# MrTornado24/FENeRF

Measured on AMD Instinct MI355X. Metric: rays/s/GPU forward render (128x128, 24+24 samples, H=256 FiLM-SIREN + 32x96^3 grid), higher is better.
Workload: dtype f16x3 (error-compensated fp16 MFMA, fp32 accumulate; fp32-class accuracy); 1 GPU; configs[1]: CelebA_double_semantic_texture_embedding_256_dim_96 generator, 128x128, 24+24 hierarchical samples, batch 1/GPU, forward-only render, procedural weights; img_size=128, num_steps=24, batch_per_gpu=1

## Files before the change

fenerf_amd/_lib.py:

```python
import ctypes as C
import os

import numpy as np

_HERE = os.path.dirname(os.path.abspath(__file__))
LIB_PATH = os.environ.get("FENERF_LIB", os.path.join(_HERE, "libfenerf_hip.so"))

ABI_VERSION = 2
MAX_GEO, MAX_COLOR, MAX_LABEL = 8, 4, 3

OK, E_INVALID, E_HIP, E_NOMEM, E_UNSUPPORTED, E_CLAMP_MODE = 0, -1, -2, -3, -4, -5
CLAMP = {"relu": 1, "softplus": 2}
FILL = {None: 0, "weight": 1, "seg_padding_background": 2, "eval_seg_padding_background": 3, "eval_white_back": 4}
FILL_COLORS = {"white": 1.0, "black": 0.0, "grey": 0.5, "light_grey": 0.81}

_fp = C.POINTER(C.c_float)
_vp = C.c_void_p


class FenerfModelDesc(C.Structure):
    _fields_ = [
        ("abi_version", C.c_int32), ("hidden_dim", C.c_int32), ("n_geo", C.c_int32), ("n_color", C.c_int32),
        ("n_label_layers", C.c_int32), ("output_dim", C.c_int32), ("grid_ch", C.c_int32),
        ("grid_d", C.c_int32), ("grid_h", C.c_int32), ("grid_w", C.c_int32), ("box_scale", C.c_float),
# ... 115 lines not shown
    "fenerf_siren_forward_save_pointwise": (_i, [_vp, _i, _i64] + [_vp] * 10),
    "fenerf_siren_backward_pointwise": (_i, [_vp, _i, _i64] + [_vp] * 9 + [_i, _vp]),
    "fenerf_siren_param_grads_pointwise": (_i, [_vp, _i, _i64] + [_vp] * 10 + [C.POINTER(FenerfSirenGrads)] + [_vp] * 2 + [_i, _vp]),
    "fenerf_siren_param_grads_fmt": (_i, [_vp, _i, _i64] + [_vp] * 9 + [_i, _vp, _vp, C.POINTER(FenerfSirenGrads), C.POINTER(FenerfSirenGrads)] + [_vp] * 3),
    "fenerf_siren_backward_stream_bytes_fmt": (_i, [_vp, _i64, _i, C.POINTER(C.c_double)]),
    "fenerf_model_set_forward_mode": (_i, [_vp, _i]),
    "fenerf_render_save_bytes": (_sz, [_vp, _i, _i, _i, _i, _i]),
    "fenerf_render_forward_save": (_i, [_vp, _i, _i, _i, _i] + [_vp] * 10 + [C.POINTER(FenerfCompositeOpts), _vp, _vp, _vp, _sz, _i, _vp]),
    "fenerf_render_backward_workspace_bytes": (_sz, [_vp, _i, _i, _i, _i, _i64, _i64]),
    "fenerf_render_backward": (_i, [_vp, _i, _i, _i, _i, _vp, _sz, _i, _vp, _vp, C.POINTER(FenerfCompositeOpts), _vp, C.POINTER(FenerfSirenGrads), _vp,
                                    C.POINTER(FenerfSirenGrads), _i64, _i64, _vp, _sz, _vp]),
    "fenerf_render_backward_split_workspace_bytes": (_sz, [_vp, _i, _i, _i, _i64, _i]),
    "fenerf_render_backward_stage": (_i, [_vp, _i, _i, _i, _i, _i, _i, _vp, _sz, _i, _vp, _vp, C.POINTER(FenerfCompositeOpts), _vp, C.POINTER(FenerfSirenGrads), _vp,
                                          C.POINTER(FenerfSirenGrads), _i64, _vp, _sz, _vp]),
    "fenerf_ray_grads": (_i, [_i, _i, _i, _i] + [_vp] * 7),
    "fenerf_render_backward_rays_workspace_bytes": (_sz, [_vp, _i, _i, _i, _i, _i, _i64, _i64]),
    "fenerf_render_backward_rays": (_i, [_vp, _i, _i, _i, _i, _vp, _sz, _i, _vp, _vp, C.POINTER(FenerfCompositeOpts), _vp, C.POINTER(FenerfSirenGrads), _vp,
                                         C.POINTER(FenerfSirenGrads), _i64, _i64, _vp, _sz, _vp, _vp, _i, _vp, _vp, _vp]),
    "fenerf_composite_backward_outputs": (_i, [_i64, _i, _i, _i, _vp, _vp, _vp, _vp, _vp, C.POINTER(FenerfCompositeOpts)] + [_vp] * 7),
    "fenerf_render_backward_outputs": (_i, [_vp, _i, _i, _i, _i, _vp, _sz, _i, _vp, _vp, C.POINTER(FenerfCompositeOpts), _vp, _vp, C.POINTER(FenerfSirenGrads),
                                            _vp, C.POINTER(FenerfSirenGrads), _i64, _i64, _vp, _sz, _vp, _vp, _i, _vp, _vp, _vp]),
    "fenerf_sparse_select_workspace_bytes": (C.c_size_t, [_i, _i64]),
    "fenerf_sparse_select": (_i, [_i, _i, _i, _i, _i64, _vp, _vp, _vp, _vp, _vp, _vp, _vp, _vp, _vp, _vp, _vp, _vp, C.c_size_t, _vp]),
    "fenerf_mesh_workspace_bytes": (_sz, [_i, _i, _i]),
    "fenerf_mesh_count": (_i, [_vp, _i, _i, _i, C.c_float, _vp, _vp, _vp]),
    "fenerf_mesh_emit": (_i, [_vp, _i, _i, _i, C.c_float, C.POINTER(C.c_float), C.POINTER(C.c_float), _vp, _i64, _i64, _vp, _vp, _vp]),
    "fenerf_volume_components_workspace_bytes": (_sz, [_i, _i, _i]),
    "fenerf_volume_components": (_i, [_vp, _i, _i, _i, C.c_float, _vp, _vp, _vp, _vp]),
    "fenerf_volume_keep_components": (_i, [_vp, _vp, _vp, _i, _i, _i, _i, _i64, _vp, _vp]),
    "fenerf_mesh_cluster_workspace_bytes": (_sz, [_i64, _i64, _i, _i, _i, _i]),
    "fenerf_mesh_cluster_count": (_i, [_vp, _i64, _vp, _i64, C.POINTER(C.c_float), C.POINTER(C.c_float), _i, _i, _i, _i, _vp, _vp, _vp]),
    "fenerf_mesh_cluster_emit": (_i, [_vp, _i64, _i64, C.POINTER(C.c_float), C.POINTER(C.c_float), _i, _i, _i, _i, _vp, _i64, _i64, _vp, _vp, _vp]),
    "fenerf_volume_sample": (_i, [_vp, _i, _i, _i, _i, _i, C.POINTER(C.c_float), C.POINTER(C.c_float), C.c_float, _i64, _vp, _vp, _vp]),
    "fenerf_volume_sample_rays": (_i, [_vp, _i, _i, _i, _i, _i, C.POINTER(C.c_float), C.POINTER(C.c_float), C.c_float, _i, _i, _i, _vp, _vp, _vp, _vp, _vp]),
    "fenerf_volume_render_workspace_bytes": (_sz, [_i, _i, _i, _i, _i]),
    "fenerf_volume_render": (_i, [_vp, _i, _i, _i, _i, _i, C.POINTER(C.c_float), C.POINTER(C.c_float), C.c_float, _i, _i, _i, _i] + [_vp] * 6 +
                             [C.POINTER(FenerfCompositeOpts)] + [_vp] * 4 + [_vp, _sz, _vp]),
    "fenerf_surface_points": (_i, [_i, _i, _vp, _vp, _vp, _vp, C.c_float, _vp, _vp]),
    "fenerf_volume_sample_grad": (_i, [_vp, _i, _i, _i, _i, _i, C.POINTER(C.c_float), C.POINTER(C.c_float), _i64, _vp, _vp, _vp]),
    "fenerf_shade_normals": (_i, [_i, _i, _i64, _vp, _vp, _vp, C.POINTER(C.c_float), C.c_float, C.c_float, C.c_float, _vp, _vp, _vp]),
    "fenerf_composite_backward": (_i, [_i64, _i, _i, _i, _vp, _vp, _vp, _vp, _vp, C.POINTER(FenerfCompositeOpts), _vp, _vp, _vp, _vp]),
    "fenerf_render_workspace_bytes": (_sz, [_vp, _i, _i, _i, _i]),
    "fenerf_render_forward": (_i, [_vp, _i, _i, _i, _i, _i] + [_vp] * 10 + [C.POINTER(FenerfCompositeOpts)] + [_vp] * 4 + [_vp, _sz, _vp]),
}
EXPORTS = tuple(_SIGS)
N_PHASES = 19
# ... 163 lines not shown
```

fenerf_amd/csrc/fenerf_api.cpp:

```cpp
#include <hip/hip_runtime.h>

#include <atomic>
#include <cmath>
#include <cstddef>
#include <cstdio>
#include <cstdlib>
#include <cstring>
#include <map>
#include <mutex>
#include <new>
#include <string>
#include <vector>

#include "fenerf_internal.h"

namespace fenerf {
static thread_local std::string g_err;
void set_error(const std::string& msg) { g_err = msg; }

int fail(int code, const std::string& msg) {
  set_error(msg);
  return code;
}
int hip_fail(hipError_t e, const char* what) {
// ... 1099 lines not shown
  p.BR = BR; p.M = M; p.C = C; p.N = N;
  p.rows_a = rows_a; p.rows_b = rows_b; p.z_a = z_a; p.z_b = z_b; p.noise = noise; p.o = *opts;
  p.g_rgb = g_rgb; p.d_rows_a = d_rows_a; p.d_rows_b = d_rows_b;
  const CompositeOutGrads g{g_depth, g_weights, g_wsum};
  { PhaseScope ph(PH_COMPOSITE_BWD, stream); return launch_composite_backward_outputs(p, g, merge != 0, stream); }
}

extern "C" size_t fenerf_sparse_select_workspace_bytes(int B, int64_t P) {
  if (B < 1 || P < 1) return 0;
  return sparse_select_workspace_bytes(B, P);
}

extern "C" int fenerf_sparse_select(int B, int R, int N, int C, int64_t cap, const float* d_coarse, const float* d_fine, const float* z_coarse,
                                    const float* z_fine, const float* origins, const float* dirs, const int64_t* images, float* pts, float* rd,
                                    float* d_sel, int32_t* counts, void* workspace, size_t workspace_bytes, void* stream) {
  if (B < 1 || B > 65535 || R < 1 || N < 1 || C < 1 || cap < 1) return fail(FENERF_E_INVALID, "need 1 <= B <= 65535, R, N, C, cap >= 1");
  if ((int64_t)R * N > (int64_t)1 << 36) return fail(FENERF_E_INVALID, "too many samples per image");
  if (!d_coarse || !z_coarse || !origins || !dirs || !pts || !d_sel || !counts || !workspace || (!d_fine) != (!z_fine))
    return fail(FENERF_E_INVALID, "NULL pointer (d_fine and z_fine may be NULL together: one pass)");
  if (workspace_bytes < sparse_select_workspace_bytes(B, (int64_t)R * N)) return fail(FENERF_E_INVALID, "workspace too small (fenerf_sparse_select_workspace_bytes)");
  { PhaseScope ph(PH_OTHER, stream); return launch_sparse_select(B, R, N, C, cap, d_coarse, d_fine, z_coarse, z_fine, origins, dirs, (const long long*)images, pts, rd, d_sel, counts, workspace, stream); }
}

namespace {
int check_lattice(const char* who, int n0, int n1, int n2) {
  if (n0 < 2 || n1 < 2 || n2 < 2) return fail(FENERF_E_INVALID, std::string(who) + ": every lattice axis needs at least 2 points");
  if ((int64_t)n0 * n1 * n2 > INT32_MAX) return fail(FENERF_E_INVALID, std::string(who) + ": more than 2^31 - 1 lattice points");
  return FENERF_OK;
}
}

extern "C" size_t fenerf_mesh_workspace_bytes(int n0, int n1, int n2) {
  if (check_lattice("fenerf_mesh_workspace_bytes", n0, n1, n2) != FENERF_OK) return 0;
  return mesh_workspace_bytes(n0, n1, n2);
}

extern "C" int fenerf_mesh_count(const float* vol, int n0, int n1, int n2, float iso, void* workspace, int64_t* counts_dev, void* stream) {
  if (int rc = check_lattice("fenerf_mesh_count", n0, n1, n2)) return rc;
  if (!vol || !workspace || !counts_dev) return fail(FENERF_E_INVALID, "fenerf_mesh_count: vol / workspace / counts_dev is NULL");
  { PhaseScope ph(PH_OTHER, stream); return launch_mesh_count(vol, n0, n1, n2, iso, workspace, (long long*)counts_dev, stream); }
}

extern "C" int fenerf_mesh_emit(const float* vol, int n0, int n1, int n2, float iso, const float origin[3], const float spacing[3], const void* workspace,
                                int64_t n_vertices, int64_t n_faces, float* vertices, int32_t* faces, void* stream) {
  if (int rc = check_lattice("fenerf_mesh_emit", n0, n1, n2)) return rc;
  if (!vol || !workspace || !origin || !spacing) return fail(FENERF_E_INVALID, "fenerf_mesh_emit: vol / workspace / origin / spacing is NULL");
// ... 173 lines not shown
  float* wts = (float*)(base + ws.wts);
  float* zf = (float*)(base + ws.zf);
  cp.BR = BR; cp.M = N; cp.C = C; cp.N = N;
  cp.rows_a = coarse; cp.z_a = z_coarse; cp.noise = noise_coarse;
  cp.o.clamp_mode = opts->clamp_mode; cp.o.noise_std = opts->noise_std;
  cp.out_weights = wts;
  cp.out_ch = C - 1; cp.sigma_only = 1;
  rc = run_composite(cp, false, stream);
  if (rc) return rc;
  { PhaseScope ph(PH_RESAMPLE, stream); rc = launch_resample(BR, N, z_coarse, wts, u, zf, stream); }
  if (rc) return rc;
  rc = run_volume_rays(vp, BR, N, origins, dirs, zf, fine, stream);
  if (rc) return rc;
  memset(&cp, 0, sizeof(cp));
  cp.BR = BR; cp.M = 2 * N; cp.C = C; cp.N = N;
  cp.rows_a = fine; cp.rows_b = coarse; cp.z_a = zf; cp.z_b = z_coarse; cp.noise = noise_final; cp.o = *opts;
  cp.out_rgb = out_rgb; cp.out_depth = out_depth; cp.out_weights = out_weights; cp.out_wsum = out_wsum;
  cp.out_ch = out_channels(C, opts);
  return run_composite(cp, true, stream);
}

namespace {
struct RenderWs {
  size_t film, coarse, fine, wts, zf, counts, idx, xbuf, total;
};
RenderWs render_ws(const FenerfModel* m, int B, int R, int N, int hier) {
  RenderWs w;
  const size_t pts = (size_t)B * R * N;
  size_t off = 0;
  w.film = off; off += fenerf_film_workspace_bytes(m, B);
  w.coarse = off; off += align_up(pts * m->C * sizeof(float), 256);
  w.fine = off; off += hier ? align_up(pts * m->C * sizeof(float), 256) : 0;
  w.wts = off; off += hier ? align_up(pts * sizeof(float), 256) : 0;
  w.zf = off; off += hier ? align_up(pts * sizeof(float), 256) : 0;
  const bool split = hier && m->precision == FENERF_PREC_F16X3;
  w.counts = off; off += split ? align_up((size_t)B * sizeof(unsigned), 256) : 0;
  w.idx = off; off += split ? align_up(pts * sizeof(unsigned), 256) : 0;
  w.xbuf = off; off += split ? align_up(pts * (size_t)m->H * sizeof(float), 256) : 0;
  w.total = off;
  return w;
}
}

extern "C" size_t fenerf_render_workspace_bytes(const FenerfModel* m, int B, int R, int N, int hierarchical) {
  if (!m || B <= 0 || R <= 0 || N <= 0) return 0;
  return render_ws(m, B, R, N, hierarchical).total;
}

extern "C" int fenerf_render_forward(const FenerfModel* m, int B, int R, int N, int hierarchical, int lock_view,
                                     const float* origins, const float* dirs, const float* z_coarse, const float* u,
                                     const float* noise_coarse, const float* noise_final, const float* freq_geo,
                                     const float* phase_geo, const float* freq_app, const float* phase_app,
                                     const FenerfCompositeOpts* opts, float* out_rgb, float* out_depth,
                                     float* out_weights, float* out_wsum, void* workspace, size_t workspace_bytes,
                                     void* stream) {
  if (!m) return fail(FENERF_E_INVALID, "model is NULL");
  int rc = check_opts(opts);
  if (rc) return rc;
  if (B <= 0 || R <= 0 || N <= 0) return fail(FENERF_E_INVALID, "B, R, N must be > 0");
  const int M = hierarchical ? 2 * N : N;
// ... 38 lines not shown
    c1.rows_a = coarse; c1.z_a = z_coarse; c1.noise = noise_coarse;
    c1.o.clamp_mode = opts->clamp_mode; c1.o.noise_std = opts->noise_std;
    c1.sigma_only = 1; c1.out_ch = m->C - 1;
    c1.u = u; c1.z_fine = zf;
    memset(&c2, 0, sizeof(c2));
    c2.BR = BR; c2.M = 2 * N; c2.C = m->C; c2.N = N;
    c2.rows_a = fine; c2.rows_b = coarse; c2.z_a = zf; c2.z_b = z_coarse; c2.noise = noise_final; c2.o = *opts;
    c2.out_rgb = out_rgb; c2.out_depth = out_depth; c2.out_weights = out_weights; c2.out_wsum = out_wsum;
    c2.out_ch = out_channels(m->C, opts);
    sp.out = coarse;
    PhaseScope ph(PH_RENDER_FUSED, stream);
    return launch_render16w_fused(m, sp, plan, zf, fine, c1, c2, stream);
  }
  const bool split_ok = m->precision == FENERF_PREC_F16X3 && m->forward_mode == FENERF_FORWARD_F16X3 && opts->clamp_mode == FENERF_CLAMP_RELU &&
                        !opts->last_back && (opts->noise_std == 0.f || !noise_final) && m->d_colour_nonfinite;
  if (g_render_split == FENERF_SPLIT_FORCE && !split_ok)
    return fail(FENERF_E_UNSUPPORTED, "fenerf_set_render_split(FORCE): the density + colour route needs an f16x3 model at its default forward mode, "
                                      "the relu clamp, last_back off and no noise on the final composite");
  const bool split = split_ok && (g_render_split == FENERF_SPLIT_FORCE || (g_render_split == FENERF_SPLIT_AUTO && kSplitAutoEnabled));
  SplitArgs sa;
  memset(&sa, 0, sizeof(sa));
  if (split) {
    sa.counts = (unsigned*)(base + ws.counts); sa.idx = (unsigned*)(base + ws.idx); sa.xbuf = (float*)(base + ws.xbuf);
    sa.cap = (long long)R * N; sa.keep_all = m->d_colour_nonfinite;
    HIP_TRY(hipMemsetAsync(sa.counts, 0, (size_t)B * sizeof(unsigned), (hipStream_t)stream));
    rc = [&] { PhaseScope ph(PH_SIREN, stream); PhaseScope pd(PH_SIREN_DENSITY, stream); return launch_siren16w_density(m, sp, sa, stream); }();
  } else {
    rc = run_siren(m, sp, stream);
  }
  if (rc) return rc;
  sp.raw_fg = nullptr;
  memset(&cp, 0, sizeof(cp));
  cp.BR = BR; cp.M = N; cp.C = m->C; cp.N = N;
  cp.rows_a = coarse; cp.z_a = z_coarse; cp.noise = noise_coarse;
  cp.o.clamp_mode = opts->clamp_mode; cp.o.noise_std = opts->noise_std;
  cp.sigma_only = 1; cp.out_ch = m->C - 1;
  cp.u = u; cp.z_fine = zf;
  rc = run_composite(cp, false, stream);
  if (rc) return rc;
  if (split) {
    rc = [&] { PhaseScope ph(PH_SIREN_COLOUR, stream); return launch_siren16w_colour(m, sp, sa, stream); }();
    if (rc) return rc;
  }
  sp.z = zf; sp.out = fine;
  rc = run_siren(m, sp, stream);
  if (rc) return rc;
  memset(&cp, 0, sizeof(cp));
  cp.BR = BR; cp.M = 2 * N; cp.C = m->C; cp.N = N;
// ... 557 lines not shown
```

fenerf_amd/csrc/fenerf_internal.h:

```cpp
#pragma once
#include <hip/hip_runtime_api.h>

#include <cstddef>
#include <cstdint>
#include <map>
#include <mutex>
#include <string>
#include <vector>

#include "../../include/fenerf.h"
#include "fenerf_layout.h"

namespace fenerf {

void set_error(const std::string& msg);
int fail(int code, const std::string& msg);
int hip_fail(hipError_t e, const char* what);
int check_launch(const char* what);
int ensure_dynamic_lds(const void* kfn, size_t bytes);
enum Phase { PH_FILM_PREP = 0, PH_SIREN, PH_SIREN_SAVE, PH_CHAIN, PH_WGRAD_FILM, PH_WGRAD_SQ, PH_WGRAD_SQ_REDUCE, PH_WGRAD_THIN,
             PH_WGRAD_THIN_REDUCE, PH_COMPOSITE, PH_RESAMPLE, PH_COMPOSITE_BWD, PH_REPACK, PH_GRID, PH_RAY_SETUP, PH_OTHER, PH_RENDER_FUSED,
             PH_SIREN_DENSITY, PH_SIREN_COLOUR, PH_COUNT };
static_assert(PH_COUNT == FENERF_N_PHASES_ALL && PH_RENDER_FUSED + 1 == FENERF_N_PHASES, "include/fenerf.h FENERF_N_PHASES / FENERF_N_PHASES_ALL");
struct PhaseScope {
// ... 125 lines not shown
int launch_siren_backward(const FenerfModel* m, const SirenBwdParams& p, void* stream);
int launch_siren_backward16w(const FenerfModel* m, const SirenBwdParams& p, void* stream);
bool use_bf16_dump(const FenerfModel* m, long long total_points);
int bwd16w_film_unit(long long total_points, long long pts_per_image);
size_t wgrad_workspace_bytes(const FenerfModel* m, int B, long long P);
int launch_param_grads(const FenerfModel* m, int B, long long P, const float* points, const float* dirs, const float* fp, const float* pp,
                       const float* out, const float* d_out, const float* tape, const float* tape_e, const float* d_t,
                       const FenerfSirenGrads& g, bool film_only, void* workspace, void* stream, const float* film_tiles = nullptr,
                       int tape_format = 0, const FenerfSirenGrads* weights = nullptr,
                       int film_per_point = 0);
int launch_grid_backward(const FenerfModel* m, long long P, const float* points, const float* d_e, float* d_grid_cl, void* stream);
size_t grid_det_workspace_bytes(const FenerfModel* m);
int launch_grid_backward_det(const FenerfModel* m, long long rows, long long dense_rows, const float* points, const float* d_e, float* out,
                             bool to_ncdhw, void* workspace, void* stream);
int launch_siren_input_grads(const FenerfModel* m, int B, long long P, const float* points, const float* fp, const float* d_t, const float* w_geo0,
                             const float* w_color0, int w_color0_ld, float* d_points, float* d_dirs, void* stream);
int launch_ray_grads(int B, int R, int N, long long Pp, int passes, const float* d_pts2, const float* d_rd2, const float* z_coarse,
                     const float* z_fine, float* d_origins, float* d_dirs, void* stream);
int launch_siren16w(const FenerfModel* m, const SirenParams& p, void* stream);
struct SplitArgs {
  unsigned* counts;
  unsigned* idx;
  float* xbuf;
  long long cap;
  const unsigned* keep_all;
};
int launch_siren16w_density(const FenerfModel* m, const SirenParams& p, const SplitArgs& s, void* stream);
int launch_siren16w_colour(const FenerfModel* m, const SirenParams& p, const SplitArgs& s, void* stream);
int launch_nonfinite_scan(FenerfModel* m, bool grid_too, void* stream);
struct FusedRenderPlan { int rays_per_group, octs_per_group, blocks; long long groups; };
bool fused_render_plan(const FenerfModel* m, long long B, long long R, int N, bool balanced_only, FusedRenderPlan* plan);
int launch_render16w_fused(const FenerfModel* m, const SirenParams& p, const FusedRenderPlan& plan, float* z_fine, float* out_fine,
                           const CompositeParams& coarse, const CompositeParams& final_, void* stream);
int launch_composite(const CompositeParams& p, bool merge, void* stream);
int launch_composite_backward(const CompositeParams& p, bool merge, void* stream);
int launch_composite_backward_outputs(const CompositeParams& p, const CompositeOutGrads& g, bool merge, void* stream);
int launch_resample(long long BR, int N, const float* z, const float* w, const float* u, float* zf, void* stream);
int launch_sample_pdf(long long BR, int K, int NS, const float* bins, const float* w, const float* u, float* out, void* stream);
int launch_ray_setup(int B, int S, int N, float z_cam, float ray_start, float ray_end, const float* u_jitter,
                     const float* theta, const float* phi, float* origins, float* dirs, float* z, float* pitch, float* yaw,
                     void* stream);
#define FENERF_MULTI_ADD_MAX 64
struct MultiAdd { float* dst[FENERF_MULTI_ADD_MAX]; const float* src[FENERF_MULTI_ADD_MAX]; long long n[FENERF_MULTI_ADD_MAX]; int count; };
struct FilmFold { float* out[4]; const float* in[4]; int row[4]; int B; };
int launch_render_points(int B, int R, int N, long long Pp, const float* origins, const float* dirs, const float* z, float* pts, float* rd, void* stream);
size_t sparse_select_workspace_bytes(int B, long long P);
int launch_sparse_select(int B, int R, int N, int C, long long cap, const float* d_coarse, const float* d_fine, const float* z_coarse,
                         const float* z_fine, const float* origins, const float* dirs, const long long* images, float* pts, float* rd, float* d_sel,
                         int* counts, void* workspace, void* stream);
size_t mesh_workspace_bytes(int n0, int n1, int n2);
const long long* mesh_workspace_totals(const void* workspace);
// ... 36 lines not shown
```

fenerf_amd/csrc/fenerf_repack.hip:

```cpp
#include <hip/hip_runtime.h>

#include <cmath>
#include <mutex>

#include "fenerf_internal.h"
#include "fenerf_layout.h"
#include "fenerf_trig.h"

namespace fenerf {

__global__ void trig_domain_kernel(const float* t, float* out, int n) {
  const int i = threadIdx.x;
  if (i < n) { out[i] = sin2pi(t[i]); out[n + i] = cos2pi(t[i]); }
}
int check_trig_domain() {
  static std::mutex mu;
  static int verdict[64] = {0};
  int dev = 0;
  hipError_t e = hipGetDevice(&dev);
  if (e != hipSuccess) { set_error(std::string("check_trig_domain: ") + hipGetErrorString(e)); return FENERF_E_HIP; }
  std::lock_guard<std::mutex> lock(mu);
  if (dev < 0 || dev >= 64) return FENERF_OK;
  if (verdict[dev] == 0) {
    const int n = 8;
// ... 115 lines not shown
  auto scan = [&](const float* p, long long n) {
    for (long long i = i0; i < n; i += stride) bad |= !(__builtin_fabsf(p[i]) < __builtin_inff());
  };
  scan(f32_a, n_a); scan(f32_b, n_b); scan(f32_c, n_c);
  for (long long i = i0; i < n_h; i += stride) bad |= (h16[i] & 0x7c00u) == 0x7c00u;
  if (bad) atomicOr(flag, 1u);
}

int launch_nonfinite_scan(FenerfModel* m, bool grid_too, void* stream) {
  if (m->precision != FENERF_PREC_F16X3 || !m->d_colour_nonfinite) return FENERF_OK;
  hipStream_t st = (hipStream_t)stream;
  hipError_t e = hipMemsetAsync(m->d_colour_nonfinite, 0, (grid_too ? 2 : 1) * sizeof(unsigned), st);
  if (e != hipSuccess) return hip_fail(e, "non-finite scan");
  const long long n_l0 = (long long)m->sh.l0_entries * 256;
  const long long n_grid = m->d_grid ? (long long)m->grid_ch * m->gd * m->gh * m->gw : 0;
  hipLaunchKernelGGL(nonfinite_scan_kernel, dim3(64), dim3(256), 0, st, m->d_stream, n_l0, m->d_consts, (long long)m->n_consts, (const float*)nullptr, 0LL,
                     reinterpret_cast<const uint16_t*>(m->d_stream + n_l0), ((long long)m->n_stream - n_l0) * 2, m->d_colour_nonfinite);
  if (grid_too && n_grid)
    hipLaunchKernelGGL(nonfinite_scan_kernel, dim3(1024), dim3(256), 0, st, m->d_grid, n_grid, (const float*)nullptr, 0LL, (const float*)nullptr, 0LL,
                       (const uint16_t*)nullptr, 0LL, m->d_colour_nonfinite + 1);
  return check_launch("non-finite scan launch");
}

}
```

fenerf_amd/csrc/fenerf_siren_f16w.hip:

```cpp
#include <hip/hip_runtime.h>

#include <type_traits>

#include "fenerf_composite_ray.h"
#include "fenerf_film.h"
#include "fenerf_internal.h"
#include "fenerf_launch.h"
#include "fenerf_layout.h"
#include "fenerf_trig.h"
#include "fenerf_wave16.h"

namespace fenerf {
namespace w16 {

using namespace wave16;

typedef _Float16 half8 __attribute__((ext_vector_type(8)));
typedef _Float16 half4 __attribute__((ext_vector_type(4)));
typedef _Float16 half2 __attribute__((ext_vector_type(2)));

#define MFMA16W(a, b, c) __builtin_amdgcn_mfma_f32_16x16x32_f16((a), (b), (c), 0, 0, 0)

__device__ __forceinline__ half8 as_half8(const float4& v) { return __builtin_bit_cast(half8, v); }
template <int MODE> struct TapeW { const char* base; };
// ... 250 lines not shown
  if constexpr (FUSED) { opg = F.octs_per_group; nunits = F.groups; }
  const int nblk = gridDim.x;
  const int nx = nblk < 8 ? nblk : 8;
  const int xcd = blockIdx.x % nx, bi = blockIdx.x / nx;
  const int blocks_in_x = nblk / nx + (xcd < nblk % nx ? 1 : 0);
  const long long o_begin = nunits * xcd / nx, o_end = nunits * (xcd + 1) / nx;

  if (P.raw_fg && o_begin + bi < o_end) {
    const long long p_first = (o_begin + bi) * opg * (NWAVE * 16);
    long long p_last = o_end * opg * (NWAVE * 16) - 1;
    if (p_last >= P.P) p_last = P.P - 1;
    film_prep_prologue(P, p_first / P.pts_per_image, p_last / P.pts_per_image, H, n_geo, n_color);
  }

#pragma unroll
  for (int i = 0; i < DPF; ++i) ws_issue(ws, i);
  wait_vmcnt<DPF - 1>();
  __builtin_amdgcn_s_barrier();
  LDS_FENCE();
  if (wave >= NWAVE / 2) __builtin_amdgcn_s_setprio(1);
  APipe a_cur;
  a_cur.c = ws_read<LOR>(ws, 0, 0);
  a_cur.n = ws_read<LOR>(ws, 0, 1);

  for (long long unit = PASS == 2 ? (long long)blockIdx.x : o_begin + bi; unit < (PASS == 2 ? c_units : o_end); unit += PASS == 2 ? nblk : blocks_in_x) {
  const int nsub = FUSED ? 2 * opg : 1;
#pragma unroll 1
  for (int sub = 0; sub < nsub; ++sub) {
    const bool fine_pass = FUSED && sub >= opg;
    const long long oct = FUSED ? unit * opg + (fine_pass ? sub - opg : sub) : unit;
    const float* z_src = P.z;
    float* out_dst = P.out;
    if constexpr (FUSED) {
      if (fine_pass) { z_src = F.z_fine; out_dst = F.out_fine; }
    }
    ws.g_next = (PASS ? g_first : g_stream) + (unsigned long long)DPF * (CH * 1024);
    const long long tile = oct * NWAVE + wave;
    long long pt = tile * 16 + n;
    if (pt >= P.P) pt = P.P - 1;
    long long c_img = 0, c_slot0 = 0;
    unsigned c_cnt = 0;
    if constexpr (PASS == 2) {
      long long u = unit;
      for (;; ++c_img) {
        c_cnt = F.counts[c_img];
        const long long nu = (c_cnt + 127u) / 128u;
// ... 24 lines not shown
    const int tile_odd = (int)(tile & 1);
    const char* tape_tile = SAVE ? uniform_ptr(reinterpret_cast<const char*>(P.tape) + (size_t)(tile >> 1) * L * TL) : nullptr;
    auto tape_of = [&](int layer) {
      TapeW<SAVE> t{SAVE ? uniform_ptr(tape_tile + (size_t)layer * TL) : nullptr};
      if (SAVE) asm volatile("s_nop 4" ::: "memory");
      return t;
    };

    const float* fp_img = P.fp + (size_t)img * L * H;
    const float* pp_img = P.pp + (size_t)img * L * H;
    auto film_issue = [&](int layer) {
      const unsigned dst = __builtin_amdgcn_readfirstlane(lds_addr(film_base) + (layer & 1) * FILM_BYTES);
      const float* gf = fp_img + (size_t)layer * H;
      const float* gp = pp_img + (size_t)layer * H;
      const unsigned vo = (unsigned)opaque(lane) * 16;
      for (int off = 0; off < H * 4; off += 1024) {
        glds_1k_s(reinterpret_cast<const char*>(gf) + off, vo, dst + off);
        glds_1k_s(reinterpret_cast<const char*>(gp) + off, vo, dst + FILM_F + off);
      }
    };
    half8 xh[KS], xl[KS];
    if constexpr (PASS == 2) {
      film_issue(n_geo);
      long long slot = c_slot0 + (opaque(lane) & 15);
      if (slot >= (long long)c_cnt) slot = (long long)c_cnt - 1;
      const float4* xb = reinterpret_cast<const float4*>(F.xbuf) + ((size_t)c_img * F.cap + slot) * (KS * 8) + (opaque(lane) >> 4);
#pragma unroll
      for (int k = 0; k < KS; ++k) { xh[k] = as_half8(xb[(2 * k + 0) * 4]); xl[k] = as_half8(xb[(2 * k + 1) * 4]); }
    } else {
    film_issue(0);
    if (L > 1) film_issue(1);
    }

    float e[8];
#pragma unroll
    for (int i = 0; i < 8; ++i) e[i] = 0.f;
    if (GRID && PASS != 1) {
      const int ch0 = 16 * (g & 1) + 8 * (g >> 1);
      const float ix = ((qx + 1.f) / 2.f) * (float)(P.gw - 1);
      const float iy = ((qy + 1.f) / 2.f) * (float)(P.gh - 1);
      const float iz = ((qz + 1.f) / 2.f) * (float)(P.gd - 1);
      const float x0 = floorf(ix), y0 = floorf(iy), z0 = floorf(iz);
#pragma unroll
      for (int c = 0; c < 8; ++c) {
        const int cz = c >> 2, cy = (c >> 1) & 1, cx = c & 1;
        const float xi = x0 + cx, yi = y0 + cy, zi = z0 + cz;
        const float wx = cx ? (ix - x0) : (x0 + 1.f - ix);
        const float wy = cy ? (iy - y0) : (y0 + 1.f - iy);
        const float wz = cz ? (iz - z0) : (z0 + 1.f - iz);
// ... 264 lines not shown
      const int n_o = lane_o & 15;
      if constexpr (PASS == 2) {
        const long long slot = c_slot0 + n_o;
        if ((lane_o >> 4) == 0 && slot < (long long)c_cnt) {
          float* row = out_dst + (c_img * P.pts_per_image + F.idx[c_img * F.cap + slot]) * C + (C - 4);
#pragma unroll
          for (int r = 0; r < 3; ++r) {
            const float v = acc[0][r] * cst[64 + r] + cst[68 + r];
            row[r] = 1.f / (1.f + __expf(-v));
          }
        }
      } else
      if ((lane_o >> 4) == 0) {
#pragma unroll
        for (int r = 0; r < 3; ++r) {
          const float v = acc[0][r] * cst[64 + r] + cst[68 + r];
          stage[n_o * C + (C - 4) + r] = 1.f / (1.f + __expf(-v));
        }
      }
    }
    __builtin_amdgcn_fence(__ATOMIC_RELEASE, "wavefront");
    __builtin_amdgcn_wave_barrier();
    __builtin_amdgcn_fence(__ATOMIC_ACQUIRE, "wavefront");
    if constexpr (PASS != 2) {
      const long long base = tile * 16 * C;
      const long long limit = P.P * C;
      for (int i = opaque(lane); i < 16 * C; i += 64)
        if (base + i < limit) out_dst[base + i] = stage[i];
    }
    if constexpr (PASS == 1) {
      const int lane_o = opaque(lane);
      const int n_o = lane_o & 15, g_o = lane_o >> 4;
      bool film_bad = false;
      for (int i = lane_o; i < n_color * H; i += 64) {
        const float fv = fp_img[(size_t)n_geo * H + i], pv = pp_img[(size_t)n_geo * H + i];
        film_bad |= !(__builtin_fabsf(fv) < __builtin_inff()) || !(__builtin_fabsf(pv) < __builtin_inff());
      }
      const bool keep_all = (F.keep_all[0] | F.keep_all[1]) != 0u || __builtin_amdgcn_ballot_w64(film_bad) != 0ull;
      const float sg = stage[n_o * C + (C - 1)];
      const long long pt_raw = tile * 16 + n_o;
      const bool keep = pt_raw < P.P && (!(sg <= 0.f) || dir_bad || keep_all);
      const unsigned long long bal = __builtin_amdgcn_ballot_w64(keep) & 0xffffull;
      const unsigned cnt = (unsigned)__builtin_popcountll(bal);
      unsigned b0 = 0;
      if (lane_o == 0 && cnt) b0 = atomicAdd(F.counts + img, cnt);
      const unsigned slot = (unsigned)__builtin_amdgcn_readfirstlane((int)b0) + (unsigned)__builtin_popcountll(bal & ((1ull << n_o) - 1ull));
      if (keep) {
        if (g_o == 0) F.idx[img * F.cap + slot] = (unsigned)(pt_raw - img * P.pts_per_image);
        float4* xb = reinterpret_cast<float4*>(F.xbuf) + ((size_t)img * F.cap + slot) * (KS * 8) + g_o;
#pragma unroll
        for (int k = 0; k < KS; ++k) {
          xb[(2 * k + 0) * 4] = __builtin_bit_cast(float4, xh[k]);
          xb[(2 * k + 1) * 4] = __builtin_bit_cast(float4, xl[k]);
        }
      }
    }
    wait_vmcnt<0>();
    __builtin_amdgcn_wave_barrier();
    if constexpr (FUSED) {
      if (FENERF_EXP_RAY_PHASE > 0 && (sub == opg - 1 || sub == nsub - 1)) {
        __builtin_amdgcn_fence(__ATOMIC_RELEASE, "workgroup");
        __builtin_amdgcn_s_barrier();
        __builtin_amdgcn_fence(__ATOMIC_ACQUIRE, "workgroup");
        float* sc = reinterpret_cast<float*>(ext_wave);
        float* s_z = sc;
        float* s_zs = sc + FUSED_MAXM;
        int* s_ord = reinterpret_cast<int*>(sc + 2 * FUSED_MAXM + 4);
        float* s_w = sc + 3 * FUSED_MAXM + 4;
        const int lane_r = opaque(lane);
        const long long ray0 = unit * F.rays_per_group;
        for (int r = wave; r < F.rays_per_group; r += NWAVE) {
          const long long ray = ray0 + r;
          if (FENERF_EXP_RAY_PHASE > 1 && ray < F.total_rays) {
#pragma unroll 1
            for (int rep = 0; rep < (FENERF_EXP_RAY_PHASE > 2 ? 2 : 1); ++rep) {
              if (!fine_pass) composite_ray<false, FUSED_MAXM>(ray_par[0], ray, lane_r, s_z, s_zs, s_ord, s_w);
              else composite_ray<true, FUSED_MAXM>(ray_par[1], ray, lane_r, s_z, s_zs, s_ord, s_w);
              __builtin_amdgcn_wave_barrier();
// ... 118 lines not shown
    q.z = p.z + (size_t)b * p.pts_per_image;
  }
  return q;
}

int launch_siren16w(const FenerfModel* m, const SirenParams& p, void* stream) {
  if (p.P <= 0) return FENERF_OK;
  if (p.pts_per_image % 32 == 0 || p.P == p.pts_per_image) return launch_siren16w_one(m, p, stream);
  const long long nimg = p.P / p.pts_per_image;
  for (long long b = 0; b < nimg; ++b) {
    int rc = launch_siren16w_one(m, image_params(m, p, b), stream);
    if (rc) return rc;
  }
  return FENERF_OK;
}

int launch_siren16w_density(const FenerfModel* m, const SirenParams& p, const SplitArgs& s, void* stream) {
  if (p.P <= 0) return FENERF_OK;
  auto one = [&](const SirenParams& q, const SplitArgs& t) {
    return dispatch_width(m->H, m->grid_ch != 0, [&](auto h, auto g) {
      return w16::launch_split_t<decltype(h)::value, decltype(g)::value, 1>(m, q, t, persistent_blocks((q.P + 15) / 16, w16::NWAVE, m->num_cus), stream);
    });
  };
  if (p.pts_per_image % 32 == 0 || p.P == p.pts_per_image) return one(p, s);
  const long long nimg = p.P / p.pts_per_image;
  for (long long b = 0; b < nimg; ++b) {
    SplitArgs t = s;
    t.counts = s.counts + b; t.idx = s.idx + (size_t)b * s.cap; t.xbuf = s.xbuf + (size_t)b * s.cap * m->H;
    int rc = one(image_params(m, p, b), t);
    if (rc) return rc;
  }
  return FENERF_OK;
}

int launch_siren16w_colour(const FenerfModel* m, const SirenParams& p, const SplitArgs& s, void* stream) {
  if (p.P <= 0) return FENERF_OK;
  const long long nimg = p.P / p.pts_per_image;
  const long long max_units = nimg * ((p.pts_per_image + 127) / 128);
  return dispatch_width(m->H, m->grid_ch != 0, [&](auto h, auto g) {
    return w16::launch_split_t<decltype(h)::value, decltype(g)::value, 2>(m, p, s, persistent_blocks(max_units, 1, m->num_cus), stream);
  });
}

}
```

fenerf_amd/native.py:

```python
import ctypes as C
import warnings

import numpy as np
import torch

from . import _lib


def _ptr(t):
    if t is None:
        return None
    assert t.is_cuda and t.dtype == torch.float32 and t.is_contiguous(), "expected a contiguous fp32 device tensor"
    return C.c_void_p(t.data_ptr())


def _stream():
    return C.c_void_p(torch.cuda.current_stream().cuda_stream)


def _f32(t, device):
    return t.detach().to(device=device, dtype=torch.float32).contiguous()


def alert_not_deterministic(what):
# ... 1133 lines not shown
    return rgb, depth, w, ws, zs


def sparse_select(d_coarse, d_fine, z_coarse, z_fine, origins, dirs, cap, want_dirs=True, images=None):
    Bin, R, _ = origins.shape
    BR, N, Cc = d_coarse.shape
    assert BR == Bin * R and cap >= 1 and (d_fine is None) == (z_fine is None) and (d_fine is None or d_fine.shape == d_coarse.shape)
    assert images is None or (images.is_cuda and images.dtype == torch.int64 and images.is_contiguous() and images.dim() == 1)
    B = Bin if images is None else images.numel()
    dev = d_coarse.device
    dc, df, zc, zf, o, d = (_f32(t, dev) if t is not None else None for t in (d_coarse, d_fine, z_coarse, z_fine, origins, dirs))
    pts = torch.empty((B, cap, 3), dtype=torch.float32, device=dev)
    rd = torch.empty((B, cap, 3), dtype=torch.float32, device=dev) if want_dirs else None
    d_sel = torch.empty((B, cap, Cc), dtype=torch.float32, device=dev)
    counts = torch.empty((B + 1,), dtype=torch.int32, device=dev)
    nbytes = _lib.lib().fenerf_sparse_select_workspace_bytes(B, R * N)
    ws = torch.empty((nbytes,), dtype=torch.uint8, device=dev)
    with torch.cuda.device(dev):
        _lib.check(_lib.lib().fenerf_sparse_select(B, R, N, Cc, cap, _ptr(dc), _ptr(df), _ptr(zc), _ptr(zf), _ptr(o), _ptr(d),
                                                   C.c_void_p(images.data_ptr()) if images is not None else None, _ptr(pts), _ptr(rd), _ptr(d_sel), C.c_void_p(counts.data_ptr()), C.c_void_p(ws.data_ptr()), nbytes, _stream()))
    return pts, rd, d_sel, counts


def ray_grads(d_points, d_viewdirs, z_coarse, z_fine=None, want_origins=True, want_dirs=True):
    B, R, N = z_coarse.shape
    passes = 1 if z_fine is None else 2
    Pp = (R * N + 31) // 32 * 32
    dev = d_points.device
    dp, zc = _f32(d_points, dev), _f32(z_coarse, dev)
    dv = _f32(d_viewdirs, dev) if d_viewdirs is not None else None
    zf = _f32(z_fine, dev) if z_fine is not None else None
    if dp.numel() != passes * B * Pp * 3 or (dv is not None and dv.numel() != dp.numel()) or (zf is not None and zf.numel() != zc.numel()):
        raise ValueError(f"ray_grads: d_points / d_viewdirs must hold [{passes} * {B}, {Pp}, 3] and z_fine as many depths as z_coarse")
    d_o = torch.empty((B, R, 3), dtype=torch.float32, device=dev) if want_origins else None
    d_d = torch.empty((B, R, 3), dtype=torch.float32, device=dev) if want_dirs else None
    with torch.cuda.device(dev):
        _lib.check(_lib.lib().fenerf_ray_grads(B, R, N, passes, _ptr(dp), _ptr(dv), _ptr(zc), _ptr(zf), _ptr(d_o), _ptr(d_d), _stream()))
    return d_o, d_d


def composite_backward(g_rgb, rows_a, z_a, opts, rows_b=None, z_b=None, noise=None, out_a=None, out_b=None, g_depth=None, g_weights=None,
                       g_wsum=None):
    BR, N, Cc = rows_a.shape
    dev = rows_a.device
    merge = rows_b is not None
    outputs = g_depth is not None or g_weights is not None or g_wsum is not None
# ... 211 lines not shown
```

include/fenerf.h:

```cpp
#ifndef FENERF_H_
#define FENERF_H_

#include <stddef.h>
#include <stdint.h>

#ifdef __cplusplus
extern "C" {
#endif

#define FENERF_ABI_VERSION 2

enum {
  FENERF_OK = 0,
  FENERF_E_INVALID = -1,
  FENERF_E_HIP = -2,
  FENERF_E_NOMEM = -3,
  FENERF_E_UNSUPPORTED = -4,
  FENERF_E_CLAMP_MODE = -5
};

enum { FENERF_PREC_F32 = 0, FENERF_PREC_F16X3 = 1 };

enum { FENERF_CLAMP_RELU = 1, FENERF_CLAMP_SOFTPLUS = 2 };

// ... 285 lines not shown
                                const float* w_color0, int w_color0_ld, float* d_origins, float* d_dirs, void* stream);

int fenerf_render_backward_outputs(const FenerfModel* m, int B, int R, int N, int lock_view, const void* save, size_t save_bytes, int tape_format,
                                   const float* z_coarse, const float* noise_final, const FenerfCompositeOpts* opts, const float* g_rgb,
                                   const float* g_depth, const FenerfSirenGrads* grads, float* d_grid_ncdhw, const FenerfSirenGrads* weights,
                                   int64_t chunk_points, int64_t film_sums_budget_bytes, void* workspace, size_t workspace_bytes,
                                   const float* w_geo0, const float* w_color0, int w_color0_ld, float* d_origins, float* d_dirs, void* stream);

int fenerf_composite_backward(int64_t BR, int N, int C, int merge, const float* rows_a, const float* rows_b,
                              const float* z_a, const float* z_b, const float* noise, const FenerfCompositeOpts* opts,
                              const float* g_rgb, float* d_rows_a, float* d_rows_b, void* stream);

int fenerf_composite_backward_outputs(int64_t BR, int N, int C, int merge, const float* rows_a, const float* rows_b,
                                      const float* z_a, const float* z_b, const float* noise, const FenerfCompositeOpts* opts,
                                      const float* g_rgb, const float* g_depth, const float* g_weights, const float* g_wsum,
                                      float* d_rows_a, float* d_rows_b, void* stream);

size_t fenerf_sparse_select_workspace_bytes(int B, int64_t P);

int fenerf_sparse_select(int B, int R, int N, int C, int64_t cap, const float* d_coarse, const float* d_fine, const float* z_coarse,
                         const float* z_fine, const float* origins, const float* dirs, const int64_t* images, float* pts, float* rd,
                         float* d_sel, int32_t* counts, void* workspace, size_t workspace_bytes, void* stream);

size_t fenerf_mesh_workspace_bytes(int n0, int n1, int n2);
int fenerf_mesh_count(const float* vol, int n0, int n1, int n2, float iso, void* workspace, int64_t* counts_dev, void* stream);
int fenerf_mesh_emit(const float* vol, int n0, int n1, int n2, float iso, const float origin[3], const float spacing[3], const void* workspace,
                     int64_t n_vertices, int64_t n_faces, float* vertices, int32_t* faces, void* stream);

#define FENERF_KEEP_LARGEST 0
#define FENERF_KEEP_MIN_POINTS 1
size_t fenerf_volume_components_workspace_bytes(int n0, int n1, int n2);
int fenerf_volume_components(const float* vol, int n0, int n1, int n2, float iso, void* workspace, int32_t* labels_dev, int64_t* stats_dev, void* stream);
int fenerf_volume_keep_components(const float* vol, const int32_t* labels, const void* workspace, int n0, int n1, int n2, int mode, int64_t min_points,
                                  float* vol_out, void* stream);
size_t fenerf_mesh_cluster_workspace_bytes(int64_t V, int64_t F, int n0, int n1, int n2, int factor);
int fenerf_mesh_cluster_count(const float* vertices, int64_t V, const int32_t* faces, int64_t F, const float origin[3], const float spacing[3], int n0, int n1,
                              int n2, int factor, void* workspace, int64_t* counts_dev, void* stream);
int fenerf_mesh_cluster_emit(const int32_t* faces, int64_t V, int64_t F, const float origin[3], const float spacing[3], int n0, int n1, int n2, int factor,
                             const void* workspace, int64_t n_vertices, int64_t n_faces, float* vertices_out, int32_t* faces_out, void* stream);

int fenerf_volume_sample(const float* vol, int n0, int n1, int n2, int C, int ld, const float origin[3], const float spacing[3],
                         float outside_last, int64_t P, const float* points, float* rows, void* stream);
int fenerf_volume_sample_rays(const float* vol, int n0, int n1, int n2, int C, int ld, const float origin[3], const float spacing[3],
                              float outside_last, int B, int R, int N, const float* origins, const float* dirs, const float* z, float* rows,
                              void* stream);
size_t fenerf_volume_render_workspace_bytes(int B, int R, int N, int C, int hierarchical);
// ... 27 lines not shown
```

Before: 6.381 million rays/s.

## Replace atomic compaction in split density pass with per-tile masks and scan

The density pass no longer uses a global atomicAdd per 16-point tile to compact kept points. It writes a 16-bit keep mask per tile and stores activations at the point's raw position. A separate scan kernel then builds the compacted index list and per-image counts, and the colour pass reads activations by raw point position. The per-image FiLM non-finite check is also cached across tiles of the same image. This removes atomic contention and the counts memset, at the cost of an extra kernel launch, an extra mask buffer, and less compact xbuf access.

```diff
diff --git a/fenerf_amd/_lib.py b/fenerf_amd/_lib.py
--- a/fenerf_amd/_lib.py
+++ b/fenerf_amd/_lib.py
@@ -161,6 +161,7 @@
                                             _vp, C.POINTER(FenerfSirenGrads), _i64, _i64, _vp, _sz, _vp, _vp, _i, _vp, _vp, _vp]),
     "fenerf_sparse_select_workspace_bytes": (C.c_size_t, [_i, _i64]),
     "fenerf_sparse_select": (_i, [_i, _i, _i, _i, _i64, _vp, _vp, _vp, _vp, _vp, _vp, _vp, _vp, _vp, _vp, _vp, _vp, C.c_size_t, _vp]),
+    "fenerf_split_scan": (_i, [_i, _i64, _i64, _vp, _vp, _vp, _vp]),
     "fenerf_mesh_workspace_bytes": (_sz, [_i, _i, _i]),
     "fenerf_mesh_count": (_i, [_vp, _i, _i, _i, C.c_float, _vp, _vp, _vp]),
     "fenerf_mesh_emit": (_i, [_vp, _i, _i, _i, C.c_float, C.POINTER(C.c_float), C.POINTER(C.c_float), _vp, _i64, _i64, _vp, _vp, _vp]),
diff --git a/fenerf_amd/csrc/fenerf_api.cpp b/fenerf_amd/csrc/fenerf_api.cpp
--- a/fenerf_amd/csrc/fenerf_api.cpp
+++ b/fenerf_amd/csrc/fenerf_api.cpp
@@ -1145,6 +1145,12 @@
   { PhaseScope ph(PH_OTHER, stream); return launch_sparse_select(B, R, N, C, cap, d_coarse, d_fine, z_coarse, z_fine, origins, dirs, (const long long*)images, pts, rd, d_sel, counts, workspace, stream); }
 }
 
+extern "C" int fenerf_split_scan(int B, int64_t tiles, int64_t cap, const uint16_t* masks, uint32_t* idx, uint32_t* counts, void* stream) {
+  if (B < 1 || B > 65535 || tiles < 1 || tiles > ((int64_t)1 << 27) || cap < 16 * tiles) return fail(FENERF_E_INVALID, "need 1 <= B <= 65535, 1 <= tiles <= 2^27, cap >= 16 tiles");
+  if (!masks || !idx || !counts) return fail(FENERF_E_INVALID, "fenerf_split_scan: masks / idx / counts is NULL");
+  { PhaseScope ph(PH_OTHER, stream); return launch_split_scan(masks, B, tiles, cap, idx, counts, stream); }
+}
+
 namespace {
 int check_lattice(const char* who, int n0, int n1, int n2) {
   if (n0 < 2 || n1 < 2 || n2 < 2) return fail(FENERF_E_INVALID, std::string(who) + ": every lattice axis needs at least 2 points");
@@ -1364,7 +1370,7 @@
 
 namespace {
 struct RenderWs {
-  size_t film, coarse, fine, wts, zf, counts, idx, xbuf, total;
+  size_t film, coarse, fine, wts, zf, counts, idx, masks, xbuf, total;
 };
 RenderWs render_ws(const FenerfModel* m, int B, int R, int N, int hier) {
   RenderWs w;
@@ -1378,6 +1384,7 @@
   const bool split = hier && m->precision == FENERF_PREC_F16X3;
   w.counts = off; off += split ? align_up((size_t)B * sizeof(unsigned), 256) : 0;
   w.idx = off; off += split ? align_up(pts * sizeof(unsigned), 256) : 0;
+  w.masks = off; off += split ? align_up((size_t)B * split_tiles_per_image((long long)R * N) * sizeof(unsigned short), 256) : 0;
   w.xbuf = off; off += split ? align_up(pts * (size_t)m->H * sizeof(float), 256) : 0;
   w.total = off;
   return w;
@@ -1462,8 +1469,8 @@
   memset(&sa, 0, sizeof(sa));
   if (split) {
     sa.counts = (unsigned*)(base + ws.counts); sa.idx = (unsigned*)(base + ws.idx); sa.xbuf = (float*)(base + ws.xbuf);
+    sa.masks = (unsigned short*)(base + ws.masks);
     sa.cap = (long long)R * N; sa.keep_all = m->d_colour_nonfinite;
-    HIP_TRY(hipMemsetAsync(sa.counts, 0, (size_t)B * sizeof(unsigned), (hipStream_t)stream));
     rc = [&] { PhaseScope ph(PH_SIREN, stream); PhaseScope pd(PH_SIREN_DENSITY, stream); return launch_siren16w_density(m, sp, sa, stream); }();
   } else {
     rc = run_siren(m, sp, stream);
diff --git a/fenerf_amd/csrc/fenerf_internal.h b/fenerf_amd/csrc/fenerf_internal.h
--- a/fenerf_amd/csrc/fenerf_internal.h
+++ b/fenerf_amd/csrc/fenerf_internal.h
@@ -171,11 +171,14 @@
   unsigned* counts;
   unsigned* idx;
   float* xbuf;
+  unsigned short* masks;
   long long cap;
   const unsigned* keep_all;
 };
+inline long long split_tiles_per_image(long long pts_per_image) { return (pts_per_image + 15) / 16; }
 int launch_siren16w_density(const FenerfModel* m, const SirenParams& p, const SplitArgs& s, void* stream);
 int launch_siren16w_colour(const FenerfModel* m, const SirenParams& p, const SplitArgs& s, void* stream);
+int launch_split_scan(const unsigned short* masks, int B, long long tiles_per_image, long long cap, unsigned* idx, unsigned* counts, void* stream);
 int launch_nonfinite_scan(FenerfModel* m, bool grid_too, void* stream);
 struct FusedRenderPlan { int rays_per_group, octs_per_group, blocks; long long groups; };
 bool fused_render_plan(const FenerfModel* m, long long B, long long R, int N, bool balanced_only, FusedRenderPlan* plan);
diff --git a/fenerf_amd/csrc/fenerf_repack.hip b/fenerf_amd/csrc/fenerf_repack.hip
--- a/fenerf_amd/csrc/fenerf_repack.hip
+++ b/fenerf_amd/csrc/fenerf_repack.hip
@@ -161,4 +161,47 @@
   return check_launch("non-finite scan launch");
 }
 
-}
+__global__ void __launch_bounds__(256) split_scan_kernel(const unsigned short* masks, long long tiles, long long cap, unsigned wgs_per_image,
+                                                         unsigned* idx, unsigned* counts) {
+  const unsigned b = blockIdx.x / wgs_per_image, piece = blockIdx.x - b * wgs_per_image;
+  const int t = threadIdx.x, lane = t & 63, w = t >> 6;
+  const unsigned short* mk = masks + (long long)b * tiles;
+  unsigned* out = idx + (long long)b * cap;
+  const long long first = (long long)piece * 256, j = first + t;
+  __shared__ unsigned wave_part[4], wave_sum[4];
+  unsigned part = 0;
+  for (long long i = t; i < first; i += 256) part += __popc((unsigned)mk[i]);
+  for (int o = 32; o; o >>= 1) part += __shfl_xor(part, o);
+  const unsigned m = j < tiles ? (unsigned)mk[j] : 0u;
+  const unsigned v = __popc(m);
+  unsigned incl = v;
+  for (int o = 1; o < 64; o <<= 1) {
+    const unsigned u = __shfl_up(incl, o);
+    if (lane >= o) incl += u;
+  }
+  if (lane == 63) wave_sum[w] = incl;
+  if (lane == 0) wave_part[w] = part;
+  __syncthreads();
+  unsigned before = wave_part[0] + wave_part[1] + wave_part[2] + wave_part[3];
+  for (int k = 0; k < w; ++k) before += wave_sum[k];
+  unsigned slot = before + incl - v;
+  for (unsigned mm = m; mm; mm &= mm - 1u) {
+    if (slot < cap) out[slot] = (unsigned)j * 16u + (unsigned)__builtin_ctz(mm);
+    ++slot;
+  }
+  if (piece == wgs_per_image - 1 && t == 255) {
+    const unsigned total = before + incl;
+    counts[b] = total < cap ? total : (unsigned)cap;
+  }
+}
+
+int launch_split_scan(const unsigned short* masks, int B, long long tiles_per_image, long long cap, unsigned* idx, unsigned* counts, void* stream) {
+  if (B <= 0 || tiles_per_image <= 0) return FENERF_OK;
+  const long long wpi = (tiles_per_image + 255) / 256;
+  if (wpi * B > 0x7fffffffLL) return fail(FENERF_E_INVALID, "split scan: more than 2^31 - 1 workgroups (images x ceil(tiles per image / 256))");
+  hipLaunchKernelGGL(split_scan_kernel, dim3((unsigned)(wpi * B)), dim3(256), 0, (hipStream_t)stream, masks, tiles_per_image, cap, (unsigned)wpi, idx,
+                     counts);
+  return check_launch("split scan launch");
+}
+
+}
diff --git a/fenerf_amd/csrc/fenerf_siren_f16w.hip b/fenerf_amd/csrc/fenerf_siren_f16w.hip
--- a/fenerf_amd/csrc/fenerf_siren_f16w.hip
+++ b/fenerf_amd/csrc/fenerf_siren_f16w.hip
@@ -296,6 +296,8 @@
   APipe a_cur;
   a_cur.c = ws_read<LOR>(ws, 0, 0);
   a_cur.n = ws_read<LOR>(ws, 0, 1);
+  [[maybe_unused]] long long chk_img = -1;
+  [[maybe_unused]] bool chk_all = false;
 
   for (long long unit = PASS == 2 ? (long long)blockIdx.x : o_begin + bi; unit < (PASS == 2 ? c_units : o_end); unit += PASS == 2 ? nblk : blocks_in_x) {
   const int nsub = FUSED ? 2 * opg : 1;
@@ -366,9 +368,7 @@
     half8 xh[KS], xl[KS];
     if constexpr (PASS == 2) {
       film_issue(n_geo);
-      long long slot = c_slot0 + (opaque(lane) & 15);
-      if (slot >= (long long)c_cnt) slot = (long long)c_cnt - 1;
-      const float4* xb = reinterpret_cast<const float4*>(F.xbuf) + ((size_t)c_img * F.cap + slot) * (KS * 8) + (opaque(lane) >> 4);
+      const float4* xb = reinterpret_cast<const float4*>(F.xbuf) + ((size_t)c_img * F.cap + (size_t)(pt - c_img * P.pts_per_image)) * (KS * 8) + (opaque(lane) >> 4);
 #pragma unroll
       for (int k = 0; k < KS; ++k) { xh[k] = as_half8(xb[(2 * k + 0) * 4]); xl[k] = as_half8(xb[(2 * k + 1) * 4]); }
     } else {
@@ -679,38 +679,37 @@
     __builtin_amdgcn_fence(__ATOMIC_RELEASE, "wavefront");
     __builtin_amdgcn_wave_barrier();
     __builtin_amdgcn_fence(__ATOMIC_ACQUIRE, "wavefront");
+    if constexpr (PASS == 1) {
+      const int lane_o = opaque(lane);
+      const int n_o = lane_o & 15, g_o = lane_o >> 4;
+      if (img != chk_img) {
+        bool film_bad = false;
+        for (int i = lane_o; i < n_color * H; i += 64) {
+          const float fv = fp_img[(size_t)n_geo * H + i], pv = pp_img[(size_t)n_geo * H + i];
+          film_bad |= !(__builtin_fabsf(fv) < __builtin_inff()) || !(__builtin_fabsf(pv) < __builtin_inff());
+        }
+        chk_all = (F.keep_all[0] | F.keep_all[1]) != 0u || __builtin_amdgcn_ballot_w64(film_bad) != 0ull;
+        chk_img = img;
+      }
+      const float sg = stage[n_o * C + (C - 1)];
+      const long long pt_raw = tile * 16 + n_o;
+      const bool keep = pt_raw < P.P && (!(sg <= 0.f) || dir_bad || chk_all);
+      const unsigned long long bal = __builtin_amdgcn_ballot_w64(keep) & 0xffffull;
+      if (keep) {
+        float4* xb = reinterpret_cast<float4*>(F.xbuf) + ((size_t)img * F.cap + (size_t)(pt_raw - img * P.pts_per_image)) * (KS * 8) + g_o;
+#pragma unroll
+        for (int k = 0; k < KS; ++k) {
+          xb[(2 * k + 0) * 4] = __builtin_bit_cast(float4, xh[k]);
+          xb[(2 * k + 1) * 4] = __builtin_bit_cast(float4, xl[k]);
+        }
+      }
+      if (lane_o == 0 && tile < ntiles) F.masks[tile] = (unsigned short)bal;
+    }
     if constexpr (PASS != 2) {
       const long long base = tile * 16 * C;
       const long long limit = P.P * C;
       for (int i = opaque(lane); i < 16 * C; i += 64)
         if (base + i < limit) out_dst[base + i] = stage[i];
-    }
-    if constexpr (PASS == 1) {
-      const int lane_o = opaque(lane);
-      const int n_o = lane_o & 15, g_o = lane_o >> 4;
-      bool film_bad = false;
-      for (int i = lane_o; i < n_color * H; i += 64) {
-        const float fv = fp_img[(size_t)n_geo * H + i], pv = pp_img[(size_t)n_geo * H + i];
-        film_bad |= !(__builtin_fabsf(fv) < __builtin_inff()) || !(__builtin_fabsf(pv) < __builtin_inff());
-      }
-      const bool keep_all = (F.keep_all[0] | F.keep_all[1]) != 0u || __builtin_amdgcn_ballot_w64(film_bad) != 0ull;
-      const float sg = stage[n_o * C + (C - 1)];
-      const long long pt_raw = tile * 16 + n_o;
-      const bool keep = pt_raw < P.P && (!(sg <= 0.f) || dir_bad || keep_all);
-      const unsigned long long bal = __builtin_amdgcn_ballot_w64(keep) & 0xffffull;
-      const unsigned cnt = (unsigned)__builtin_popcountll(bal);
-      unsigned b0 = 0;
-      if (lane_o == 0 && cnt) b0 = atomicAdd(F.counts + img, cnt);
-      const unsigned slot = (unsigned)__builtin_amdgcn_readfirstlane((int)b0) + (unsigned)__builtin_popcountll(bal & ((1ull << n_o) - 1ull));
-      if (keep) {
-        if (g_o == 0) F.idx[img * F.cap + slot] = (unsigned)(pt_raw - img * P.pts_per_image);
-        float4* xb = reinterpret_cast<float4*>(F.xbuf) + ((size_t)img * F.cap + slot) * (KS * 8) + g_o;
-#pragma unroll
-        for (int k = 0; k < KS; ++k) {
-          xb[(2 * k + 0) * 4] = __builtin_bit_cast(float4, xh[k]);
-          xb[(2 * k + 1) * 4] = __builtin_bit_cast(float4, xl[k]);
-        }
-      }
     }
     wait_vmcnt<0>();
     __builtin_amdgcn_wave_barrier();
@@ -875,15 +874,18 @@
       return w16::launch_split_t<decltype(h)::value, decltype(g)::value, 1>(m, q, t, persistent_blocks((q.P + 15) / 16, w16::NWAVE, m->num_cus), stream);
     });
   };
-  if (p.pts_per_image % 32 == 0 || p.P == p.pts_per_image) return one(p, s);
-  const long long nimg = p.P / p.pts_per_image;
-  for (long long b = 0; b < nimg; ++b) {
-    SplitArgs t = s;
-    t.counts = s.counts + b; t.idx = s.idx + (size_t)b * s.cap; t.xbuf = s.xbuf + (size_t)b * s.cap * m->H;
-    int rc = one(image_params(m, p, b), t);
-    if (rc) return rc;
-  }
-  return FENERF_OK;
+  const long long nimg = p.P / p.pts_per_image, tpi = split_tiles_per_image(p.pts_per_image);
+  if (p.pts_per_image % 32 == 0 || p.P == p.pts_per_image) {
+    if (int rc = one(p, s)) return rc;
+  } else {
+    for (long long b = 0; b < nimg; ++b) {
+      SplitArgs t = s;
+      t.masks = s.masks + (size_t)b * tpi; t.xbuf = s.xbuf + (size_t)b * s.cap * m->H;
+      int rc = one(image_params(m, p, b), t);
+      if (rc) return rc;
+    }
+  }
+  return launch_split_scan(s.masks, (int)nimg, tpi, s.cap, s.idx, s.counts, stream);
 }
 
 int launch_siren16w_colour(const FenerfModel* m, const SirenParams& p, const SplitArgs& s, void* stream) {
diff --git a/fenerf_amd/native.py b/fenerf_amd/native.py
--- a/fenerf_amd/native.py
+++ b/fenerf_amd/native.py
@@ -1179,6 +1179,17 @@
     return pts, rd, d_sel, counts
 
 
+def split_scan(masks, cap=None):
+    assert masks.is_cuda and masks.dtype == torch.int16 and masks.dim() == 2 and masks.is_contiguous()
+    B, tiles = masks.shape
+    cap = 16 * tiles if cap is None else cap
+    idx = torch.full((B, cap), -1, dtype=torch.int32, device=masks.device)
+    counts = torch.empty((B,), dtype=torch.int32, device=masks.device)
+    with torch.cuda.device(masks.device):
+        _lib.check(_lib.lib().fenerf_split_scan(B, tiles, cap, C.c_void_p(masks.data_ptr()), C.c_void_p(idx.data_ptr()), C.c_void_p(counts.data_ptr()), _stream()))
+    return idx, counts
+
+
 def ray_grads(d_points, d_viewdirs, z_coarse, z_fine=None, want_origins=True, want_dirs=True):
     B, R, N = z_coarse.shape
     passes = 1 if z_fine is None else 2
diff --git a/include/fenerf.h b/include/fenerf.h
--- a/include/fenerf.h
+++ b/include/fenerf.h
@@ -331,6 +331,8 @@
                          const float* z_fine, const float* origins, const float* dirs, const int64_t* images, float* pts, float* rd,
                          float* d_sel, int32_t* counts, void* workspace, size_t workspace_bytes, void* stream);
 
+int fenerf_split_scan(int B, int64_t tiles, int64_t cap, const uint16_t* masks, uint32_t* idx, uint32_t* counts, void* stream);
+
 size_t fenerf_mesh_workspace_bytes(int n0, int n1, int n2);
 int fenerf_mesh_count(const float* vol, int n0, int n1, int n2, float iso, void* workspace, int64_t* counts_dev, void* stream);
 int fenerf_mesh_emit(const float* vol, int n0, int n1, int n2, float iso, const float origin[3], const float spacing[3], const void* workspace,
```

New measurement: 6.465 million rays/s, median of 6. 1.3% higher.
